# TencentARC/ViT-Lens

Hardware: AMD Instinct MI355X
Metric: modality-pairs/sec (ViT-L, 224^2 patches) (higher is better)
Workload: dtype bf16; 1 GPU; C3: ViT-L Lens(depth)->ViT + image + text tri-modal InfoNCE TRAINING step (fwd+bwd+AdamW), batch 1024/GPU in micro-batches of 256, first 4 blocks + adapter trainable; global_batch=1024, residual_dtype=bf16, accumulate=fp32, parallelism=dp1, gemm_cfg=-1, via=step, text_tower_operands=fp16, layernorm=folded into the GEMMs (frozen blocks), frozen_towers=second HIP stream beside the trainable tower's forward, backward=two halves of the micro-batches on two HIP streams

## Files before the change

include/vitlens_hip.h:

```cpp
#ifndef VITLENS_HIP_H
#define VITLENS_HIP_H

#include <stdint.h>

#ifdef __cplusplus
extern "C" {
#endif

#ifndef __HIP_PLATFORM_AMD__
typedef struct ihipStream_t* hipStream_t;
#endif

#define VL_EPI_BF16 0
#define VL_EPI_F32 1
#define VL_EPI_RES_F32 2
#define VL_EPI_RES_BF16 3
#define VL_EPI_GEGLU 5
#define VL_EPI_DGELU 6
#define VL_EPI_DGEGLU 7
#define VL_ACT_NONE 0
#define VL_ACT_GELU 1
#define VL_ACT_RELU 2
#define VL_ACT_GELU_DSAVE 4
#define VL_ACT_QGELU 5
// ... 100 lines not shown
int vl_transpose_to_bf16(const void* in, int in_dtype, long ldi, int R, int C, void* out, long ldo, hipStream_t stream);
int vl_transpose_colsum_bf16(const void* in, int in_dtype, long ldi, int R, int C, void* out, long ldo,
                             float* colsum_out, float colsum_scale, float* ws, hipStream_t stream);

int vl_split_bf16x3(const float* x, void* out, long rows, int D, int pattern, hipStream_t stream);
int vl_ce_stats(const float* logits, long ld, int R, int C, int label_off, float* row_lse, float* col_lse,
                float* diag, float* col_ws, hipStream_t stream);
int vl_ce_loss_accum(const float* row_lse, const float* col_lse, const float* diag, int R, int C, int label_off,
                     float w_row, float w_col, float* loss_inout, hipStream_t stream);
int vl_ce_grad(const float* logits, long ld, int R, int C, int label_off, const float* row_lse, const float* col_lse,
               float w_row, float w_col, void* G, long ldg, void* GT, long ldgt, float logit_scale,
               float* dscale_inout, float* ws, hipStream_t stream);
long vl_ce_grad_ws_floats(int R, int C, long ldg, long ldgt);
int vl_ce_stats_masked(const float* logits, long ld, int R, int C, int label_off, float* row_lse, float* col_lse,
                       float* diag, float* col_ws, const float* sim, long ld_sim, float thres, hipStream_t stream);
int vl_ce_grad_masked(const float* logits, long ld, int R, int C, int label_off, const float* row_lse, const float* col_lse,
                      float w_row, float w_col, void* G, long ldg, void* GT, long ldgt, float logit_scale,
                      float* dscale_inout, float* ws, const float* sim, long ld_sim, float thres, hipStream_t stream);

int vl_layernorm_bwd(const void* dy, int dy_dtype, long dy_stride, const void* x, int x_dtype, long x_stride,
                     const float* mean, const float* rstd, const float* w, const float* dres, float* dx,
                     void* dx_bf16, long dx_stride, int rows, int D, hipStream_t stream);
int vl_layernorm_bwd_g(const void* dy, int dy_dtype, long dy_stride, const void* x, int x_dtype, long x_stride,
                       const float* mean, const float* rstd, const float* w, const void* dres, void* dx, int g_dtype,
                       void* dx_bf16, long dx_stride, int rows, int D, hipStream_t stream);
int vl_layernorm_bwd_sres(const void* dy, int dy_dtype, long dy_stride, const void* x, int x_dtype, long x_stride,
                          const float* mean, const float* rstd, const float* w, const void* dres, int dres_every,
                          long dres_stride, void* dx, int g_dtype, void* dx_bf16, long dx_stride, int rows, int D,
                          hipStream_t stream);
long vl_colreduce_ws_floats(int rows, int cols, int planes);
int vl_layernorm_bwd_params(const void* dy, int dy_dtype, long dy_stride, const void* x, int x_dtype, long x_stride,
                            const float* mean, const float* rstd, float* dw, float* db, int rows, int D,
                            float* ws, hipStream_t stream);
int vl_colsum(const void* a, int a_dtype, long lda, float* out, int rows, int cols, float scale, float* ws, hipStream_t stream);
int vl_gelu_bf16(const void* u, void* y, long n, hipStream_t stream);
int vl_geglu_bf16(const void* h, void* y, long rows, int n_out, hipStream_t stream);
int vl_attn_bwd_bf16(const void* q, const void* k, const void* v, const void* dO, const void* o, const long* strides,
                     const float* lse, float* delta, void* dq, void* dk, void* dv, long ld_dq, long ld_dkv,
                     int B, int H, int Lq, int Lk, int dh, float qscale, int causal, float scale, hipStream_t stream);
int vl_attn_bwd_fused_supported(int Lq, int Lk, int dh, int causal);
int vl_attn_bwd_fused_bf16(const void* q, const void* k, const void* v, const void* dO, const void* o, const long* strides,
                           const float* lse, void* dq, void* dk, void* dv, long ld_dq, long ld_dkv, int B, int H, int L, int dh,
                           float qscale, float scale, hipStream_t stream);
int vl_attn_fwd_q1(const void* q, const void* k, const void* v, const long* strides, void* out, long ld_out, float* lse,
                   int B, int H, int L, int dh, int qrow, float qscale, hipStream_t stream);
int vl_attn_bwd_q1(const void* q, const void* k, const void* v, const long* strides, const void* dO, long ld_do,
                   const void* o, long ld_o, const float* lse, void* dq, void* dk, void* dv, long ld_dq, long ld_dkv,
                   int B, int H, int L, int dh, int qrow, float qscale, float scale, hipStream_t stream);
int vl_attn_fwd_drop_bf16(const void* q, const void* k, const void* v, const long* strides, void* out, float* lse, int B, int H,
                          int Lq, int Lk, int dh, float qscale, int causal, double p, uint64_t seed, int64_t sample0,
                          int sublayer, hipStream_t stream);
int vl_attn_bwd_drop_bf16(const void* q, const void* k, const void* v, const void* dO, const void* o, const long* strides,
                          const float* lse, float* delta, void* dq, void* dk, void* dv, long ld_dq, long ld_dkv, int B, int H,
                          int Lq, int Lk, int dh, float qscale, int causal, float scale, double p, uint64_t seed,
                          int64_t sample0, int sublayer, hipStream_t stream);
int vl_ff_drop_fwd(const float* y, const float* x0, float* x1, int B, int n, int D, double p, uint64_t seed, int64_t sample0,
                   int sublayer, hipStream_t stream);
int vl_ff_drop_bwd(const float* dx1, void* dy, float* dy_f32, int B, int n, int D, double p, uint64_t seed, int64_t sample0,
                   int sublayer, hipStream_t stream);
int vl_kaldi_fbank(const float* wave, long wave_stride, int batch, long n_samples, const float* window, const float* banks,
                   float* out, int target_len, int win, int shift, int nfft, int nmel, float preemph, float mean, float std,
                   hipStream_t stream);
int vl_resample_sinc(const float* in, long in_stride, int batch, long n_in, const int* offsets, const float* taps, int o, int n,
                     int K, float* out, long out_stride, long out_first, long n_out, hipStream_t stream);
int vl_fbank_augment(const float* in, float* out, int batch, int T, int F, const void* params, float mean, float std,
                     hipStream_t stream);
// ... 112 lines not shown
```

vit-lens_amd/csrc/vl_bwd.hip:

```cpp
#include "vl_common.h"
#include "vitlens_hip.h"

namespace {

__device__ __forceinline__ float ld1(const float* p) { return *p; }
__device__ __forceinline__ float ld1(const bf16_t* p) { return bf2f(*p); }

__device__ __forceinline__ void ld4(const float* p, float (&v)[4]) {
  const f32x4 t = *(const f32x4*)p; v[0] = t[0]; v[1] = t[1]; v[2] = t[2]; v[3] = t[3];
}
__device__ __forceinline__ void ld4(const bf16_t* p, float (&v)[4]) {
  const u32x2 t = *(const u32x2*)p;
  v[0] = bf2f((bf16_t)(t[0] & 0xffff)); v[1] = bf2f((bf16_t)(t[0] >> 16));
  v[2] = bf2f((bf16_t)(t[1] & 0xffff)); v[3] = bf2f((bf16_t)(t[1] >> 16));
}
__device__ __forceinline__ void st4(float* p, const float (&v)[4]) { f32x4 t = {v[0], v[1], v[2], v[3]}; *(f32x4*)p = t; }
__device__ __forceinline__ void st4(bf16_t* p, const float (&v)[4]) {
  u32x2 t; t[0] = pack2bf(v[0], v[1]); t[1] = pack2bf(v[2], v[3]); *(u32x2*)p = t;
}

struct LnBwdP {
  const void* dy; const void* x; const float* mean; const float* rstd; const float* w;
  const void* dres;
  void* dx; bf16_t* dxb;
// ... 41 lines not shown
    }
    s1 = wave_sum(s1) / (float)D; s2 = wave_sum(s2) / (float)D;
#pragma unroll
    for (int c = 0; c < NV; ++c) {
      if (HALF && c == NCH && !tail) break;
      const int e = c * 256 + lane * 4;
      float v[4];
#pragma unroll
      for (int k = 0; k < 4; ++k) v[k] = rs * (g[c][k] - s1 - xh[c][k] * s2);
      if (dres) {
        float r[4]; ld4(dres + e, r);
#pragma unroll
        for (int k = 0; k < 4; ++k) v[k] += r[k];
      }
      if (dx) st4(dx + e, v);
      if (dxb) st4(dxb + e, v);
    }
  } else {
    float s1 = 0.f, s2 = 0.f;
    for (int e = lane; e < D; e += 64) {
      const float g = ld1(dy + e) * p.w[e];
      const float xh = (ld1(x + e) - mu) * rs;
      s1 += g; s2 = fmaf(g, xh, s2);
    }
    s1 = wave_sum(s1) / (float)D; s2 = wave_sum(s2) / (float)D;
    for (int e = lane; e < D; e += 64) {
      const float g = ld1(dy + e) * p.w[e];
      const float xh = (ld1(x + e) - mu) * rs;
      float v = rs * (g - s1 - xh * s2);
      if (dres) v += ld1(dres + e);
      if (dx) { if constexpr (sizeof(TG) == 4) dx[e] = v; else dx[e] = f2bf(v); }
      if (dxb) dxb[e] = f2bf(v);
    }
  }
}

__global__ void __launch_bounds__(256) gelu_kernel(const bf16_t* u, bf16_t* y, long n) {
  for (long i = ((long)blockIdx.x * 256 + threadIdx.x) * 8; i < n; i += (long)gridDim.x * 256 * 8) {
    const u32x4 v = *(const u32x4*)(u + i);
    u32x4 o;
#pragma unroll
    for (int e = 0; e < 4; ++e)
      o[e] = pack2bf(gelu_erf(bf2f((bf16_t)(v[e] & 0xffff))), gelu_erf(bf2f((bf16_t)(v[e] >> 16))));
    *(u32x4*)(y + i) = o;
  }
}

__global__ void __launch_bounds__(256) geglu_kernel(const bf16_t* h, bf16_t* y, long n) {
  for (long i = ((long)blockIdx.x * 256 + threadIdx.x) * 4; i < n; i += (long)gridDim.x * 256 * 4) {
    const u32x4 v = *(const u32x4*)(h + 2 * i);
    u32x2 o;
    o[0] = pack2bf(bf2f((bf16_t)(v[0] & 0xffff)) * gelu_erf(bf2f((bf16_t)(v[0] >> 16))),
                   bf2f((bf16_t)(v[1] & 0xffff)) * gelu_erf(bf2f((bf16_t)(v[1] >> 16))));
    o[1] = pack2bf(bf2f((bf16_t)(v[2] & 0xffff)) * gelu_erf(bf2f((bf16_t)(v[2] >> 16))),
                   bf2f((bf16_t)(v[3] & 0xffff)) * gelu_erf(bf2f((bf16_t)(v[3] >> 16))));
    *(u32x2*)(y + i) = o;
  }
}

struct AdamwC { float lr, b1, b2, eps, bc1, bc2_sqrt; };
__device__ __forceinline__ void adamw_update(float& pi, const float gi, float& mi, float& vi, const AdamwC c, const float wd) {
#pragma clang fp contract(off)
  const float decay = fmaf(-c.lr, wd, 1.0f);
  mi = fmaf(1.0f - c.b1, gi, c.b1 * mi);
  vi = c.b2 * vi + ((1.0f - c.b2) * gi) * gi;
  pi = pi * decay - ((c.lr / c.bc1) * mi) / (sqrtf(vi) / c.bc2_sqrt + c.eps);
// ... 177 lines not shown
  else if (vec && p.D == 256) hipLaunchKernelGGL((ln_bwd_kernel<1, TDY, TX, TG>), g, b, 0, stream, p);
  else hipLaunchKernelGGL((ln_bwd_kernel<0, TDY, TX, TG>), g, b, 0, stream, p);
}

static int ln_bwd_run(const void* dy, int dy_dtype, long dy_stride, const void* x, int x_dtype, long x_stride,
                      const float* mean, const float* rstd, const float* w, const void* dres, int dres_every, long dres_stride,
                      void* dx, int g_dtype, void* dx_bf16, long dx_stride, int rows, int D, hipStream_t stream) {
  if (rows <= 0 || D <= 0) return vl_set_error("vl_layernorm_bwd: empty problem");
  for (const int dt : {dy_dtype, x_dtype, g_dtype})
    if (dt != VL_F32 && dt != VL_BF16) return vl_set_error("vl_layernorm_bwd: dy_dtype, x_dtype and g_dtype must be VL_F32 or VL_BF16");
  LnBwdP p{dy, x, mean, rstd, w, dres, dx, (bf16_t*)dx_bf16, dy_stride, x_stride, dx_stride, rows, D, dres_every, dres_stride};
  const int key = (dy_dtype == VL_BF16 ? 4 : 0) | (x_dtype == VL_BF16 ? 2 : 0) | (g_dtype == VL_BF16 ? 1 : 0);
  switch (key) {
    case 0: ln_bwd_launch<float, float, float>(p, stream); break;
    case 1: ln_bwd_launch<float, float, bf16_t>(p, stream); break;
    case 2: ln_bwd_launch<float, bf16_t, float>(p, stream); break;
    case 3: ln_bwd_launch<float, bf16_t, bf16_t>(p, stream); break;
    case 4: ln_bwd_launch<bf16_t, float, float>(p, stream); break;
    case 5: ln_bwd_launch<bf16_t, float, bf16_t>(p, stream); break;
    case 6: ln_bwd_launch<bf16_t, bf16_t, float>(p, stream); break;
    default: ln_bwd_launch<bf16_t, bf16_t, bf16_t>(p, stream); break;
  }
  VL_HIP_OK(hipGetLastError());
  return 0;
}

extern "C" int vl_layernorm_bwd_g(const void* dy, int dy_dtype, long dy_stride, const void* x, int x_dtype, long x_stride,
                                  const float* mean, const float* rstd, const float* w, const void* dres, void* dx, int g_dtype,
                                  void* dx_bf16, long dx_stride, int rows, int D, hipStream_t stream) {
  return ln_bwd_run(dy, dy_dtype, dy_stride, x, x_dtype, x_stride, mean, rstd, w, dres, 1, dx_stride, dx, g_dtype, dx_bf16, dx_stride,
                    rows, D, stream);
}

extern "C" int vl_layernorm_bwd_sres(const void* dy, int dy_dtype, long dy_stride, const void* x, int x_dtype, long x_stride,
                                     const float* mean, const float* rstd, const float* w, const void* dres, int dres_every,
                                     long dres_stride, void* dx, int g_dtype, void* dx_bf16, long dx_stride, int rows, int D,
                                     hipStream_t stream) {
  if (!dres || !dx || dres_every < 1) return vl_set_error("vl_layernorm_bwd_sres: dres, dx and dres_every >= 1 are required");
  if (dres == dx) return vl_set_error("vl_layernorm_bwd_sres: dres must not alias dx");
  return ln_bwd_run(dy, dy_dtype, dy_stride, x, x_dtype, x_stride, mean, rstd, w, dres, dres_every, dres_stride, dx, g_dtype, dx_bf16,
                    dx_stride, rows, D, stream);
}

extern "C" int vl_layernorm_bwd(const void* dy, int dy_dtype, long dy_stride, const void* x, int x_dtype, long x_stride,
                                const float* mean, const float* rstd, const float* w, const float* dres, float* dx,
                                void* dx_bf16, long dx_stride, int rows, int D, hipStream_t stream) {
  return vl_layernorm_bwd_g(dy, dy_dtype, dy_stride, x, x_dtype, x_stride, mean, rstd, w, dres, dx, VL_F32, dx_bf16, dx_stride, rows, D, stream);
}

extern "C" int vl_gelu_bf16(const void* u, void* y, long n, hipStream_t stream) {
  if (n <= 0) return 0;
  if (n & 7) return vl_set_error("vl_gelu_bf16: n must be a multiple of 8");
  hipLaunchKernelGGL(gelu_kernel, dim3(grid_for(n / 8)), dim3(256), 0, stream, (const bf16_t*)u, (bf16_t*)y, n);
  VL_HIP_OK(hipGetLastError());
  return 0;
}

extern "C" int vl_geglu_bf16(const void* h, void* y, long rows, int n_out, hipStream_t stream) {
  const long n = rows * n_out;
  if (n <= 0) return 0;
  if (n_out & 3) return vl_set_error("vl_geglu_bf16: n_out must be a multiple of 4");
  hipLaunchKernelGGL(geglu_kernel, dim3(grid_for(n / 4)), dim3(256), 0, stream, (const bf16_t*)h, (bf16_t*)y, n);
  VL_HIP_OK(hipGetLastError());
  return 0;
}

// ... 69 lines not shown
```

vit-lens_amd/csrc/vl_colreduce.hip:

```cpp
#include "vl_common.h"
#include "vitlens_hip.h"

namespace {

template <int V, typename T>
__device__ __forceinline__ void ldv(const T* p, float (&f)[V]) {
  constexpr bool kF32 = sizeof(T) == 4;
  static_assert(V == 1 || (kF32 ? V == 4 : V == 4 || V == 8), "no load of this width");
  if constexpr (V == 1) {
    if constexpr (kF32) f[0] = *p; else f[0] = bf2f(*p);
  } else if constexpr (kF32) {
    const f32x4 v = *(const f32x4*)p;
#pragma unroll
    for (int e = 0; e < 4; ++e) f[e] = v[e];
  } else {
    typedef __attribute__((ext_vector_type(V / 2))) unsigned int words_t;
    const words_t v = *(const words_t*)p;
#pragma unroll
    for (int e = 0; e < V / 2; ++e) { f[2 * e] = bf2f((bf16_t)(v[e] & 0xffff)); f[2 * e + 1] = bf2f((bf16_t)(v[e] >> 16)); }
  }
}

template <int V, int NR, int U, bool LN, typename TA, typename TX>
__global__ void __launch_bounds__(256) colreduce_kernel(const TA* a, long lda, const TX* x, long xs, const float* mean,
// ... 71 lines not shown
  if (j < D) {
    for (int r = r0 + ry; r < r1; r += 8) {
      const bool two = r + 4 < r1;
      const int r2 = two ? r + 4 : r;
      const u32x2 g0 = *(const u32x2*)(dy + (long)r * dys + j), g1 = *(const u32x2*)(dy + (long)r2 * dys + j);
      const f32x4 x0 = *(const f32x4*)(x + (long)r * xs + j), x1 = *(const f32x4*)(x + (long)r2 * xs + j);
      const float m0 = mean[r], s0 = rstd[r], m1 = mean[r2], s1 = two ? rstd[r2] : 0.f;
      const float k1 = two ? 1.f : 0.f;
#pragma unroll
      for (int e = 0; e < 4; ++e) {
        const float gl = bf2f((bf16_t)((e & 1) ? (g0[e >> 1] >> 16) : (g0[e >> 1] & 0xffff)));
        const float hl = bf2f((bf16_t)((e & 1) ? (g1[e >> 1] >> 16) : (g1[e >> 1] & 0xffff)));
        a[e] = fmaf(gl, (x0[e] - m0) * s0, a[e]);
        b[e] += gl;
        a[e] = fmaf(hl, (x1[e] - m1) * s1, a[e]);
        b[e] = fmaf(hl, k1, b[e]);
      }
    }
  }
  if (ry) {
#pragma unroll
    for (int e = 0; e < 4; ++e) { sh[ry - 1][cx][e] = a[e]; sh[ry - 1][cx][4 + e] = b[e]; }
  }
  __syncthreads();
  if (ry == 0 && j < D) {
#pragma unroll
    for (int e = 0; e < 4; ++e) {
      ws[((long)blockIdx.y * 2) * D + j + e] = (a[e] + sh[0][cx][e]) + (sh[1][cx][e] + sh[2][cx][e]);
      ws[((long)blockIdx.y * 2 + 1) * D + j + e] = (b[e] + sh[0][cx][4 + e]) + (sh[1][cx][4 + e] + sh[2][cx][4 + e]);
    }
  }
}

__global__ void __launch_bounds__(1024) slab_finalize_kernel(const float* ws, int nslab, int K, int D, float scale, float* out0, float* out1) {
  __shared__ float sh[16][64];
  const int jl = threadIdx.x & 63, g = threadIdx.x >> 6;
  const int j = blockIdx.x * 64 + jl, k = blockIdx.y;
  float s = 0.f;
  if (j < D)
    for (int t = g; t < nslab; t += 16) s += ws[((long)t * K + k) * D + j];
  sh[g][jl] = s;
  __syncthreads();
  if (g == 0 && j < D) {
    float a[16];
#pragma unroll
    for (int i = 0; i < 16; ++i) a[i] = sh[i][jl];
#pragma unroll
    for (int w = 8; w > 0; w >>= 1)
#pragma unroll
      for (int i = 0; i < w; ++i) a[i] += a[i + w];
    float* o = k == 0 ? out0 : out1;
    o[j] += a[0] * scale;
  }
}

}

extern "C" int vl_set_error(const char* msg);
#define VL_HIP_OK(e) do { hipError_t _e = (e); if (_e != hipSuccess) return vl_set_error(hipGetErrorString(_e)); } while (0)

static const int kSlabRows = 256;
extern "C" long vl_colreduce_ws_floats(int rows, int cols, int planes) {
  return (long)((rows + kSlabRows - 1) / kSlabRows) * planes * cols;
}

template <typename T>
static bool vec_ok(int V, const void* p, long stride, int cols) {
  return cols % V == 0 && stride % V == 0 && (uintptr_t)p % (V * sizeof(T)) == 0;
}

template <int V, int NR, int U, bool LN, typename TA, typename TX>
static void stage1_launch(const void* a, long lda, const void* x, long xs, const float* mean, const float* rstd, float* ws,
                          int rows, int cols, int nslab, hipStream_t stream) {
  constexpr int per_block = 256 / NR * V;
  hipLaunchKernelGGL((colreduce_kernel<V, NR, U, LN, TA, TX>), dim3((cols + per_block - 1) / per_block, nslab), dim3(256), 0, stream,
                     (const TA*)a, lda, (const TX*)x, xs, mean, rstd, ws, rows, cols, kSlabRows);
}

template <int V, bool LN, typename TA, typename TX>
static void colreduce_launch(const void* a, long lda, const void* x, long xs, const float* mean, const float* rstd, float* ws,
                             int rows, int cols, float scale, float* out0, float* out1, hipStream_t stream) {
  const int nslab = (rows + kSlabRows - 1) / kSlabRows;
  bool vec = false;
  if constexpr (V > 1) {
    vec = vec_ok<TA>(V, a, lda, cols) && (!LN || vec_ok<TX>(V, x, xs, cols));
    if constexpr (LN && V == 4) {
      if (vec)
        hipLaunchKernelGGL(ln_bwd_params4_bf16_f32_kernel, dim3((cols + 255) / 256, nslab), dim3(256), 0, stream, (const bf16_t*)a, lda,
                           (const float*)x, xs, mean, rstd, ws, rows, cols, kSlabRows);
    } else if (vec) {
      stage1_launch<V, 4, LN ? 2 : 4, LN, TA, TX>(a, lda, x, xs, mean, rstd, ws, rows, cols, nslab, stream);
    }
  }
  if (!vec) stage1_launch<1, 1, 1, LN, TA, TX>(a, lda, x, xs, mean, rstd, ws, rows, cols, nslab, stream);
  hipLaunchKernelGGL(slab_finalize_kernel, dim3((cols + 63) / 64, LN ? 2 : 1), dim3(1024), 0, stream, ws, nslab, LN ? 2 : 1, cols,
                     scale, out0, out1);
}

extern "C" int vl_layernorm_bwd_params(const void* dy, int dy_dtype, long dy_stride, const void* x, int x_dtype, long x_stride,
                                       const float* mean, const float* rstd, float* dw, float* db, int rows, int D,
                                       float* ws, hipStream_t stream) {
  if (rows <= 0 || D <= 0) return vl_set_error("vl_layernorm_bwd_params: empty problem");
  if (!ws) return vl_set_error("vl_layernorm_bwd_params: workspace of vl_colreduce_ws_floats(rows, D, 2) floats required");
#define VL_LN_PARAMS(V, TA, TX) colreduce_launch<V, true, TA, TX>(dy, dy_stride, x, x_stride, mean, rstd, ws, rows, D, 1.0f, dw, db, stream)
  if (dy_dtype == VL_BF16 && x_dtype == VL_F32) VL_LN_PARAMS(4, bf16_t, float);
  else if (dy_dtype == VL_BF16) VL_LN_PARAMS(8, bf16_t, bf16_t);
  else if (x_dtype == VL_F32) VL_LN_PARAMS(1, float, float);
  else VL_LN_PARAMS(1, float, bf16_t);
#undef VL_LN_PARAMS
  VL_HIP_OK(hipGetLastError());
  return 0;
}

extern "C" int vl_colsum(const void* a, int a_dtype, long lda, float* out, int rows, int cols, float scale, float* ws, hipStream_t stream) {
  if (rows <= 0 || cols <= 0) return vl_set_error("vl_colsum: empty problem");
  if (!ws) return vl_set_error("vl_colsum: workspace of vl_colreduce_ws_floats(rows, cols, 1) floats required");
  if (a_dtype == VL_BF16) colreduce_launch<8, false, bf16_t, bf16_t>(a, lda, nullptr, 0, nullptr, nullptr, ws, rows, cols, scale, out, out, stream);
  else colreduce_launch<4, false, float, float>(a, lda, nullptr, 0, nullptr, nullptr, ws, rows, cols, scale, out, out, stream);
  VL_HIP_OK(hipGetLastError());
  return 0;
}
```

vit-lens_amd/vitlens_hip/_lib.py:

```python
import ctypes as C
import os

_HERE = os.path.dirname(os.path.abspath(__file__))
_LIB = None


class LibraryNotBuilt(ImportError):
    pass


def lib_path() -> str:
    return os.path.join(_HERE, "libvitlens_hip.so")


P, I, L, F = C.c_void_p, C.c_int, C.c_long, C.c_float

ABI_VERSION = 610

SIGNATURES = {
    "vl_version": [],
    "vl_device_info": [I, C.c_char_p, I, C.POINTER(I), C.POINTER(I), C.POINTER(L)],
    "vl_gemm_bf16": [P, P, P, P, P, I, I, I, I, I, I, F, I, I, I, P],
    "vl_gemm_splitk_accum_f32": [P, P, P, I, I, I, I, I, L, F, I, P, P],
    "vl_gemm_tn_splitk_accum_f32": [P, P, P, I, I, I, I, I, L, F, I, P, P],
# ... 42 lines not shown
    "vl_fbank_augment": [P, P, I, I, I, P, F, F, P],
    "vl_wave_clip_mix": [P, L, P, P, P, I, L, P],
    "vl_mix_rows": [P, P, P, P, P, I, L, P],
    "vl_fps": [P, P, P, P, I, I, I, P],
    "vl_pc_gather_normalize": [P, P, P, I, I, I, I, P],
    "vl_pc_augment": [P, P, P, I, I, I, I, P, F, P],
    "vl_rgbd_augment": [P, I, I, I, P, P, P, P, F, F, F, P, P, P],
    "vl_image_crop_resize_u8": [P, I, I, I, P, P, P, P],
    "vl_image_augment": [P, I, I, I, I, P, P, P, P, P, P, P, P],
    "vl_tactile_augment": [P, I, I, I, P, P, P, P, P, P],
    "vl_resample_h_u8": [P, L, I, I, I, I, P, P, I, I, I, P, P],
    "vl_resample_v_u8_norm": [P, I, I, I, I, P, P, I, I, I, P, P, P, P, P],
    "vl_resample_batch_u8_norm": [P, I, I, I, I, I, P, P, P, P, P, P],
    "vl_resample_h_f32": [P, L, I, I, I, P, P, I, I, I, I, F, F, F, P, P],
    "vl_resample_v_f32_norm": [P, I, I, I, P, P, I, I, I, F, F, P, P],
    "vl_knn_group": [P, P, P, P, I, I, I, I, I, P],
    "vl_ball_group": [P, P, P, P, P, I, I, I, I, F, I, I, P],
    "vl_group_max": [P, L, P, I, L, L, I, I, P],
    "vl_pad3_bf16": [P, P, L, I, P],
    "vl_bn_stats": [P, L, I, I, P, I, P, P, P, P, F, P],
    "vl_bn_stats_local": [P, L, I, I, P, I, P, P],
    "vl_bn_stats_merge": [P, I, I, P, P, P, P, F, P, P],
    "vl_bn_bwd_reduce": [P, L, P, L, P, P, P, P, F, I, P, I, P, P, P, I, I, P],
    "vl_bn_bwd_apply": [P, L, P, L, P, P, P, P, F, I, P, P, P, L, I, I, P],
    "vl_bn_apply": [P, L, P, P, P, P, F, I, P, L, L, I, P],
    "vl_bn_bwd": [P, L, P, L, P, P, P, P, F, I, I, P, I, P, P, P, L, I, I, P],
    "vl_group_max_bwd": [P, L, P, L, P, L, P, L, L, I, I, P],
    "vl_group_sum": [P, L, P, L, L, I, I, P],
    "vl_layernorm_bwd": [P, I, L, P, I, L, P, P, P, P, P, P, L, I, I, P],
    "vl_layernorm_bwd_g": [P, I, L, P, I, L, P, P, P, P, P, I, P, L, I, I, P],
    "vl_layernorm_bwd_sres": [P, I, L, P, I, L, P, P, P, P, I, L, P, I, P, L, I, I, P],
    "vl_colreduce_ws_floats": [I, I, I],
    "vl_layernorm_bwd_params": [P, I, L, P, I, L, P, P, P, P, I, I, P, P],
    "vl_colsum": [P, I, L, P, I, I, F, P, P],
    "vl_gelu_bf16": [P, P, L, P],
    "vl_geglu_bf16": [P, P, L, I, P],
    "vl_attn_bwd_bf16": [P, P, P, P, P, P, P, P, P, P, P, L, L, I, I, I, I, I, F, I, F, P],
    "vl_attn_bwd_fused_supported": [I, I, I, I],
    "vl_attn_bwd_fused_bf16": [P, P, P, P, P, P, P, P, P, P, L, L, I, I, I, I, F, F, P],
    "vl_attn_fwd_q1": [P, P, P, P, P, L, P, I, I, I, I, I, F, P],
    "vl_attn_bwd_q1": [P, P, P, P, P, L, P, L, P, P, P, P, L, L, I, I, I, I, I, F, F, P],
    "vl_adamw_step": [P, P, P, P, L, F, F, F, F, F, I, F, P],
    "vl_sumsq_ws_floats": [],
    "vl_sumsq_f32": [P, L, P, P, P],
    "vl_adamw_multi_step": [P, I, F, F, F, F, I, F, F, P, P, P],
    "vl_clamp_scalar": [P, F, F, P],
    "vl_axpy_f32": [P, P, F, L, P],
    "vl_scale_exp_f32": [P, P, L, P, F, P],
    "vl_batch_rowsum": [P, P, I, I, I, L, L, P],
    "vl_attn_fwd_drop_bf16": [P, P, P, P, P, P, I, I, I, I, I, F, I, C.c_double, C.c_uint64, C.c_int64, I, P],
    "vl_attn_bwd_drop_bf16": [P, P, P, P, P, P, P, P, P, P, P, L, L, I, I, I, I, I, F, I, F, C.c_double, C.c_uint64, C.c_int64, I, P],
    "vl_ff_drop_fwd": [P, P, P, I, I, I, C.c_double, C.c_uint64, C.c_int64, I, P],
    "vl_ff_drop_bwd": [P, P, P, I, I, I, C.c_double, C.c_uint64, C.c_int64, I, P],
    "vl_lp_bn_fwd": [P, L, P, F, C.c_uint64, C.c_int64, I, P, P, F, F, P, L, P, L, P, P, I, I, P],
    "vl_ce_label_ws_floats": [I, I],
    "vl_ce_label": [P, L, P, I, I, F, P, P, L, P, L, P, P, P],
    "vl_lars_ws_floats": [L, I],
    "vl_lars_multi_step": [P, I, F, F, F, F, F, P, P, L, P],
    "vl_topk_hits": [P, L, P, I, I, I, I, P, P, P],
    "vl_eval_hits": [P, L, P, P, I, I, I, I, P, P, P, P, P, P],
    "vl_average_precision_ws_bytes": [I, I],
    "vl_average_precision": [P, L, P, L, I, I, P, P, P],
    "vl_clip_mean_normalize": [P, L, I, I, I, F, P, P],
    "vl_comm_unique_id": [P],
    "vl_comm_create": [C.POINTER(P), P, I, I],
    "vl_comm_destroy": [P],
# ... 44 lines not shown
```

vit-lens_amd/vitlens_hip/ops.py:

```python
import ctypes as C
import threading

import numpy as np
import torch

from ._lib import load_library, check

F32, BF16, F16 = 0, 1, 2
EPI_BF16, EPI_F32, EPI_RES_F32, EPI_RES_BF16, EPI_GEGLU, EPI_DGELU, EPI_DGEGLU = 0, 1, 2, 3, 5, 6, 7
ACT_NONE, ACT_GELU, ACT_RELU = 0, 1, 2
ACT_GELU_DSAVE = 4
ACT_QGELU = 5
ACT_QGELU_DSAVE = 6


def mlp_act(quick_gelu: bool, dsave: bool = False) -> int:
    if quick_gelu:
        return ACT_QGELU_DSAVE if dsave else ACT_QGELU
    return ACT_GELU_DSAVE if dsave else ACT_GELU
LOG2E = 1.4426950408889634

_lib = load_library()


# ... 629 lines not shown
                                     sim.stride(0), float(thres), _stream()))
    return G, GT


def device_info(device=0):
    arch = C.create_string_buffer(64)
    cus, clk, mem = C.c_int(), C.c_int(), C.c_long()
    check(_lib.vl_device_info(device, arch, 64, C.byref(cus), C.byref(clk), C.byref(mem)))
    return {"arch": arch.value.decode(), "cus": cus.value, "clock_khz": clk.value, "hbm_bytes": mem.value}


def layernorm_bwd(dy, x, mean, rstd, w, rows, D, dres=None, dx=None, dx_bf16=None, x_row_stride=None,
                  dy_row_stride=None, dx_row_stride=None):
    g = dx if dx is not None else dres
    gdt = F32 if g is None else _dt(g)
    if dres is not None and dx is not None and dres.dtype != dx.dtype:
        raise TypeError("layernorm_bwd: dres and dx must share a dtype")
    check(_lib.vl_layernorm_bwd_g(_p(dy), _dt(dy), D if dy_row_stride is None else dy_row_stride, _p(x), _dt(x),
                                  D if x_row_stride is None else x_row_stride, _p(mean), _p(rstd), _p(w), _p(dres),
                                  _p(dx), gdt, _p(dx_bf16), D if dx_row_stride is None else dx_row_stride, rows, D, _stream()))


def layernorm_bwd_sparse_res(dy, x, mean, rstd, w, rows, D, dres, dres_every, dx):
    if dres.dtype != dx.dtype or dres.dim() != 2 or dres.stride(1) != 1 or dres.shape[0] * dres_every < rows - dres_every + 1:
        raise ValueError("layernorm_bwd_sparse_res: dres must be a row-major matrix of dx's dtype with one row per dres_every rows")
    check(_lib.vl_layernorm_bwd_sres(_p(dy), _dt(dy), D, _p(x), _dt(x), D, _p(mean), _p(rstd), _p(w), _p(dres), int(dres_every),
                                     dres.stride(0), _p(dx), _dt(dx), None, D, rows, D, _stream()))


_colreduce_ws = {}


def _ws_for(device, rows, cols, planes):
    need = int(_lib.vl_colreduce_ws_floats(rows, cols, planes))
    key = (device, torch.cuda.current_stream(device).cuda_stream, threading.get_ident())
    t = _colreduce_ws.get(key)
    if t is None or t.numel() < need:
        t = torch.empty(need, device=device, dtype=torch.float32)
        _colreduce_ws[key] = t
    return t


def layernorm_bwd_params(dy, x, mean, rstd, dw, db, rows, D, x_row_stride=None, dy_row_stride=None):
    ws = _ws_for(dy.device, rows, D, 2)
    check(_lib.vl_layernorm_bwd_params(_p(dy), _dt(dy), D if dy_row_stride is None else dy_row_stride, _p(x), _dt(x),
                                       D if x_row_stride is None else x_row_stride, _p(mean), _p(rstd), _p(dw), _p(db),
                                       rows, D, _p(ws), _stream()))


def colsum(a, out, scale=1.0):
    _chk2d(a, "a")
    ws = _ws_for(a.device, a.shape[0], a.shape[1], 1)
    check(_lib.vl_colsum(_p(a), _dt(a), a.stride(0), _p(out), a.shape[0], a.shape[1], float(scale), _p(ws), _stream()))


def geglu_bf16(h, out):
    check(_lib.vl_geglu_bf16(_p(h), _p(out), h.shape[0], h.shape[1] // 2, _stream()))
    return out


def gelu_bf16(u, out):
    check(_lib.vl_gelu_bf16(_p(u), _p(out), u.numel(), _stream()))
    return out


def attn_bwd(q, k, v, dO, o, lse, delta, dq, dk, dv, ld_dq, ld_dkv, causal=False, softmax_scale=None, qscale=None, fused=None):
    B, H, Lq, dh = q.shape
    Lk = k.shape[2]
    scale = dh ** -0.5 if softmax_scale is None else softmax_scale
    qs = scale * LOG2E if qscale is None else qscale
    st = _bhld_strides(q, k, v, dO, o)
    if fused is None:
        fused = bool(_lib.vl_attn_bwd_fused_supported(Lq, Lk, dh, 1 if causal else 0))
    if fused:
        if Lq != Lk or causal:
            raise ValueError("attn_bwd(fused=True): self-attention without a causal mask only")
        check(_lib.vl_attn_bwd_fused_bf16(_p(q), _p(k), _p(v), _p(dO), _p(o), st, _p(lse), _p(dq), _p(dk), _p(dv),
                                          ld_dq, ld_dkv, B, H, Lq, dh, float(qs), float(scale), _stream()))
        return
    check(_lib.vl_attn_bwd_bf16(_p(q), _p(k), _p(v), _p(dO), _p(o), st, _p(lse), _p(delta), _p(dq), _p(dk), _p(dv),
# ... 756 lines not shown
```

vit-lens_amd/vitlens_hip/train.py:

```python
from typing import Dict, Iterable, Optional

import torch

from . import ops
from . import engine as _engine
from .engine import VitEngine, deinterleave_geglu

BF = torch.bfloat16


class _Saved:

    def __init__(self, B, L, D, H, hidden, layers, device, res_dtype=torch.float32, keep_blocks=(), checkpoint=False):
        dh = D // H
        T = B * L
        Lp = (L + 7) // 8 * 8
        f32 = lambda *s: torch.empty(*s, device=device, dtype=torch.float32)
        bf = lambda *s: torch.empty(*s, device=device, dtype=BF)
        self.Lp = Lp
        xres = f32 if res_dtype == torch.float32 else bf

        def per_layer(make):
            if not checkpoint:
                return [make() for _ in range(layers)]
            one = make()
            return [one] * layers
        mids = per_layer(lambda: xres(T, D))
        self.X = [None] * (2 * layers + 1)
        for l in range(layers):
            self.X[2 * l] = xres(T, D); self.X[2 * l + 1] = mids[l]
        self.X[2 * layers] = xres(T, D)
        ident = lambda: [torch.zeros(T, device=device), torch.ones(T, device=device), torch.zeros(T, device=device),
                         torch.ones(T, device=device)]
        self.stats = per_layer(ident)
        self.qkv = per_layer(lambda: bf(T, 3 * D))
        hv = lambda m, i=0: ops.heads_view(m, B, L, H, dh, i * D)
        self.q = [hv(m, 0) for m in self.qkv]; self.k = [hv(m, 1) for m in self.qkv]; self.v = [hv(m, 2) for m in self.qkv]
        self.a = per_layer(lambda: bf(T, D))
        self.av = [hv(m) for m in self.a]
        self.lse = per_layer(lambda: f32(B, H, L))
        self.u = per_layer(lambda: bf(T, hidden))
# ... 163 lines not shown
        if self._drop is not None:
            dtok = ops.scatter_rows_keep(dxpre, self._drop[1], L - 1)
            if self.train_pos:
                gpos = self.grad_buffer(P + "positional_embedding", e.pos)
                ops.batch_rowsum(dxpre, gpos[:1], B, 1, D, L, 0)
                ops.batch_rowsum(dtok, gpos[1:], B, T, D, T, 0)
            return dtok
        if self.train_pos:
            ops.batch_rowsum(dxpre, self.grad_buffer(P + "positional_embedding", e.pos), B, L, D, L, 0)
        return dxpre.view(B, L, D)[:, 1:, :].reshape(B * T, D)

    def _cls_block_backward(self, S, l, B, L):
        e, D = self.eng, self.D
        w, wT, cfg = e.blocks[l], self.wT[l], e.gemm_cfg
        m1, r1 = S.stats[l][0], S.stats[l][1]
        x1c = _engine.cls_rows(S.X[2 * l + 1], B, L)
        ops.gemm(S.dxc, wT["proj_w"], None, out=S.du1, res=S.u1, epi=ops.EPI_DGELU, act=self.act_dsave, cfg=cfg)
        ops.gemm(S.du1, wT["fc_w"], None, out=S.dhc, epi=ops.EPI_BF16, cfg=cfg)
        ops.layernorm_bwd(S.dhc, x1c, S.stats2c[0], S.stats2c[1], w["ln2_w"], B, D, dres=S.dxc, dx=S.dxc, x_row_stride=L * D)
        ops.gemm(S.dxc, wT["out_w"], None, out=S.dO1, epi=ops.EPI_BF16, cfg=cfg)
        ops.attn_bwd_q1(S.q[l], S.k[l], S.v[l], S.dO1, S.a1, S.lse1, S.dqkv, S.dqkv[:, D:], S.dqkv[:, 2 * D:], 3 * D, 3 * D, qrow=0)
        ops.gemm(S.dqkv, wT["in_w"], None, out=S.dh, epi=ops.EPI_BF16, cfg=cfg)
        ops.layernorm_bwd_sparse_res(S.dh, S.X[2 * l], m1, r1, w["ln1_w"], B * L, D, dres=S.dxc, dres_every=L, dx=S.dx)

    def _blocks_backward(self, S, B, L, on_block_done=None, cls_only=False):
        e, D, H = self.eng, self.D, self.H
        rows = B * L
        cfg = e.gemm_cfg
        P = self.prefix
        f32_stream = S.dx.dtype == torch.float32
        dxb_out = S.dxb if f32_stream else None
        if f32_stream:
            ops.cast_bf16(S.dx, out=S.dxb)
        for l in reversed(range(self.layers)):
            if cls_only and l == self.layers - 1:
                self._cls_block_backward(S, l, B, L)
                continue
            if self.checkpoint:
                self._block_forward(S, l, B, L, write_out=False)
            w, wT = e.blocks[l], self.wT[l]
            m1, r1, m2, r2 = S.stats[l]
            trainable = l in self.train_blocks
            bp = f"{P}transformer.resblocks.{l}."
            ops.gemm(S.dxb, wT["proj_w"], None, out=S.du, res=S.u[l], epi=ops.EPI_DGELU, act=self.act_dsave, cfg=cfg)
            if trainable:
                self._dw(bp + "mlp.c_proj.weight", S.dx, S.hidk[l], bp + "mlp.c_proj.bias")
                self._dw(bp + "mlp.c_fc.weight", S.du, S.h2[l], bp + "mlp.c_fc.bias")
            ops.gemm(S.du, wT["fc_w"], None, out=S.dh, epi=ops.EPI_BF16, cfg=cfg)
            if trainable:
                ops.layernorm_bwd_params(S.dh, S.X[2 * l + 1], m2, r2, self.grad_buffer(bp + "ln_2.weight", w["ln2_w"]),
                                         self.grad_buffer(bp + "ln_2.bias", w["ln2_b"]), rows, D)
            ops.layernorm_bwd(S.dh, S.X[2 * l + 1], m2, r2, w["ln2_w"], rows, D, dres=S.dx, dx=S.dx, dx_bf16=dxb_out)
            if trainable:
                self._dw(bp + "attn.out_proj.weight", S.dx, S.a[l], bp + "attn.out_proj.bias")
            ops.gemm(S.dxb, wT["out_w"], None, out=S.dOm, epi=ops.EPI_BF16, cfg=cfg)
            ops.attn_bwd(S.q[l], S.k[l], S.v[l], S.dO, S.av[l], S.lse[l], S.delta,
                         S.dqkv, S.dqkv[:, D:], S.dqkv[:, 2 * D:], 3 * D, 3 * D, causal=self.causal)
            if trainable:
                self._dw(bp + "attn.in_proj_weight", S.dqkv, S.h1[l], bp + "attn.in_proj_bias")
            ops.gemm(S.dqkv, wT["in_w"], None, out=S.dh, epi=ops.EPI_BF16, cfg=cfg)
            if trainable:
                ops.layernorm_bwd_params(S.dh, S.X[2 * l], m1, r1, self.grad_buffer(bp + "ln_1.weight", w["ln1_w"]),
                                         self.grad_buffer(bp + "ln_1.bias", w["ln1_b"]), rows, D)
            ops.layernorm_bwd(S.dh, S.X[2 * l], m1, r1, w["ln1_w"], rows, D, dres=S.dx, dx=S.dx, dx_bf16=dxb_out)
            if trainable and on_block_done is not None:
                on_block_done(l)


def conv_weight_grad(dtok: torch.Tensor, cols: torch.Tensor, g: torch.Tensor, gemm_cfg: int = -1):
    ops.weight_grad(ops.cast_bf16(dtok.contiguous()), cols, g, cfg=gemm_cfg)


class DepthLensTrainer:

    def __init__(self, lens_engine, unlock_first_n: int = 4, tower_kw=None):
        self.le = lens_engine
        kw = dict(train_blocks=range(unlock_first_n)) if tower_kw is None else dict(tower_kw)
        self.tower = TowerTrainer(lens_engine.vit, param_prefix="visual.", **kw)
        self.ctx = None

    @property
    def grads(self):
        return self.tower.grads

    def forward(self, x: torch.Tensor, keep=None, inv=None) -> torch.Tensor:
        le = self.le
        cols = le.cols(x)
        tok = ops.gemm(cols, le.conv_w, None, epi=ops.EPI_BF16, cfg=le.gemm_cfg)
        self.ctx = (cols, x.shape[0])
        return self.tower.forward(tok, x.shape[0], pos2=le.adapter_pos, keep=keep, inv=inv)

    def backward(self, dfeat: torch.Tensor, on_block_done=None):
        cols, B = self.ctx
        dtok = self.tower.backward(dfeat, on_block_done)
        T, D = dtok.shape[0] // B, dtok.shape[1]
        t = self.tower
        g = t.grad_buffer("visual.visual_adapter.conv1.weight_gemm", torch.empty(D, cols.shape[1]))
# ... 451 lines not shown
```

Baseline: 1884 modality-pairs/sec.

## Fuse LayerNorm backward with its param-grad and next bias column sums

Adds a single LayerNorm-backward kernel that writes dx and, in the same pass, accumulates per-column partial sums for ln weight/bias grads and the column sum of the resulting dx. That dx column sum is the bias grad of the preceding linear layer (out_proj or the block below's c_proj). The trainer uses it for trainable blocks, so the separate layernorm_bwd_params pass and the bias column reductions inside _dw are skipped. This cuts extra reads of dy, x and dx over all rows. In exchange it adds a partial-sum workspace, a finalize launch, and bookkeeping across blocks for which c_proj bias was already produced.

```diff
diff --git a/include/vitlens_hip.h b/include/vitlens_hip.h
--- a/include/vitlens_hip.h
+++ b/include/vitlens_hip.h
@@ -156,6 +156,10 @@
 int vl_layernorm_bwd_params(const void* dy, int dy_dtype, long dy_stride, const void* x, int x_dtype, long x_stride,
                             const float* mean, const float* rstd, float* dw, float* db, int rows, int D,
                             float* ws, hipStream_t stream);
+int vl_layernorm_bwd_sums_parts(int rows, int D);
+int vl_layernorm_bwd_sums(const void* dy, long dy_stride, const void* x, int x_dtype, long x_stride, const float* mean,
+                          const float* rstd, const float* w, const void* dres, void* dx, int g_dtype, void* dx_bf16,
+                          long dx_stride, float* dw, float* db, float* dcol, int rows, int D, float* ws, hipStream_t stream);
 int vl_colsum(const void* a, int a_dtype, long lda, float* out, int rows, int cols, float scale, float* ws, hipStream_t stream);
 int vl_gelu_bf16(const void* u, void* y, long n, hipStream_t stream);
 int vl_geglu_bf16(const void* h, void* y, long rows, int n_out, hipStream_t stream);
diff --git a/vit-lens_amd/csrc/vl_bwd.hip b/vit-lens_amd/csrc/vl_bwd.hip
--- a/vit-lens_amd/csrc/vl_bwd.hip
+++ b/vit-lens_amd/csrc/vl_bwd.hip
@@ -97,6 +97,97 @@
       if (dx) { if constexpr (sizeof(TG) == 4) dx[e] = v; else dx[e] = f2bf(v); }
       if (dxb) dxb[e] = f2bf(v);
     }
+  }
+}
+
+constexpr int kLnSumsWaves = 4;
+template <typename T> struct Raw4 { typedef f32x4 type; };
+template <> struct Raw4<bf16_t> { typedef u32x2 type; };
+template <int NCH, typename TX, typename TG>
+__global__ void __launch_bounds__(kLnSumsWaves * 64) __attribute__((amdgpu_waves_per_eu(3))) ln_bwd_sums_kernel(const LnBwdP p, float* ws, const int want) {
+#pragma clang fp contract(off)
+  __shared__ float sh[kLnSumsWaves - 1][NCH * 256];
+  const int lane = threadIdx.x & 63, wv = threadIdx.x >> 6;
+  const long gw = (long)blockIdx.x * kLnSumsWaves + wv, nw = (long)gridDim.x * kLnSumsWaves;
+  const int r0 = (int)(gw * p.rows / nw), r1 = (int)((gw + 1) * p.rows / nw);
+  const int D = p.D;
+  const bool round_dx = sizeof(TG) == 2 || !p.dx;
+  float acc[3][NCH][4];
+#pragma unroll
+  for (int a = 0; a < 3; ++a)
+#pragma unroll
+    for (int c = 0; c < NCH; ++c)
+#pragma unroll
+      for (int k = 0; k < 4; ++k) acc[a][c][k] = 0.f;
+  for (int row = r0; row < r1; ++row) {
+    const bf16_t* dy = (const bf16_t*)p.dy + (long)row * p.dys;
+    const TX* x = (const TX*)p.x + (long)row * p.xs;
+    const TG* dres = p.dres ? (const TG*)p.dres + (long)row * p.dxs : nullptr;
+    TG* dx = p.dx ? (TG*)p.dx + (long)row * p.dxs : nullptr;
+    bf16_t* dxb = p.dxb ? p.dxb + (long)row * p.dxs : nullptr;
+    const float mu = p.mean[row], rs = p.rstd[row];
+    float g[NCH][4], xh[NCH][4], d0[4], w0[4];
+    float s1 = 0.f, s2 = 0.f;
+    typename Raw4<TG>::type rr[NCH];
+    if (dres) {
+#pragma unroll
+      for (int c = 0; c < NCH; ++c) rr[c] = *(const typename Raw4<TG>::type*)(dres + c * 256 + lane * 4);
+    }
+#pragma unroll
+    for (int c = 0; c < NCH; ++c) {
+      const int e = c * 256 + lane * 4;
+      float d[4], ww[4];
+      ld4(dy + e, d); ld4(x + e, xh[c]); ld4(p.w + e, ww);
+#pragma unroll
+      for (int k = 0; k < 4; ++k) {
+        g[c][k] = d[k] * ww[k]; xh[c][k] = (xh[c][k] - mu) * rs;
+        s1 += g[c][k]; s2 = fmaf(g[c][k], xh[c][k], s2);
+        acc[0][c][k] = fmaf(d[k], xh[c][k], acc[0][c][k]); acc[1][c][k] += d[k];
+        if (c == 0) { d0[k] = d[k]; w0[k] = ww[k]; }
+      }
+    }
+    s1 = wave_sum(s1) / (float)D; s2 = wave_sum(s2) / (float)D;
+#pragma unroll
+    for (int c = 0; c < NCH; ++c) {
+      const int e = c * 256 + lane * 4;
+      float v[4];
+#pragma unroll
+      for (int k = 0; k < 4; ++k) v[k] = rs * fmaf(-s2, xh[c][k], c == 0 ? fmaf(d0[k], w0[k], -s1) : g[c][k] - s1);
+      if (dres) {
+        float r[4]; ld4((const TG*)&rr[c], r);
+#pragma unroll
+        for (int k = 0; k < 4; ++k) v[k] += r[k];
+      }
+      if (dx) st4(dx + e, v);
+      if (dxb) st4(dxb + e, v);
+#pragma unroll
+      for (int k = 0; k < 4; ++k) acc[2][c][k] += round_dx ? bf2f(f2bf(v[k])) : v[k];
+    }
+  }
+  int slot = 0;
+#pragma unroll
+  for (int a = 0; a < 3; ++a) {
+    if (!(want >> a & 1)) continue;
+    if (wv > 0) {
+#pragma unroll
+      for (int c = 0; c < NCH; ++c) st4(&sh[wv - 1][c * 256 + lane * 4], acc[a][c]);
+    }
+    __syncthreads();
+    if (wv == 0) {
+      float* out = ws + ((long)blockIdx.x * __popc(want) + slot) * D;
+#pragma unroll
+      for (int c = 0; c < NCH; ++c) {
+        float s[4] = {acc[a][c][0], acc[a][c][1], acc[a][c][2], acc[a][c][3]};
+        for (int w = 0; w < kLnSumsWaves - 1; ++w) {
+          float t[4]; ld4(&sh[w][c * 256 + lane * 4], t);
+#pragma unroll
+          for (int k = 0; k < 4; ++k) s[k] += t[k];
+        }
+        st4(out + c * 256 + lane * 4, s);
+      }
+    }
+    __syncthreads();
+    ++slot;
   }
 }
 
@@ -340,6 +431,56 @@
                     rows, D, stream);
 }
 
+void vl_colreduce_finalize(const float* ws, int nparts, int planes, int cols, float* out0, float* out1, float* out2, hipStream_t stream);
+
+extern "C" int vl_layernorm_bwd_sums_parts(int rows, int D) {
+  if (rows <= 0 || D <= 0 || D % 256 != 0 || D > 1024) return 0;
+  const int n = (rows + kLnSumsWaves - 1) / kLnSumsWaves;
+  return n > 768 ? 768 : n;
+}
+
+template <typename TX, typename TG>
+static void ln_bwd_sums_launch(const LnBwdP& p, float* ws, int want, int nparts, hipStream_t stream) {
+  const dim3 g(nparts), b(kLnSumsWaves * 64);
+  switch (p.D / 256) {
+    case 1: hipLaunchKernelGGL((ln_bwd_sums_kernel<1, TX, TG>), g, b, 0, stream, p, ws, want); break;
+    case 2: hipLaunchKernelGGL((ln_bwd_sums_kernel<2, TX, TG>), g, b, 0, stream, p, ws, want); break;
+    case 3: hipLaunchKernelGGL((ln_bwd_sums_kernel<3, TX, TG>), g, b, 0, stream, p, ws, want); break;
+    default: hipLaunchKernelGGL((ln_bwd_sums_kernel<4, TX, TG>), g, b, 0, stream, p, ws, want); break;
+  }
+}
+
+extern "C" int vl_layernorm_bwd_sums(const void* dy, long dy_stride, const void* x, int x_dtype, long x_stride, const float* mean,
+                                     const float* rstd, const float* w, const void* dres, void* dx, int g_dtype, void* dx_bf16,
+                                     long dx_stride, float* dw, float* db, float* dcol, int rows, int D, float* ws,
+                                     hipStream_t stream) {
+  const int nparts = vl_layernorm_bwd_sums_parts(rows, D);
+  if (nparts == 0) return vl_set_error("vl_layernorm_bwd_sums: D must be 256, 512, 768 or 1024 and rows > 0 (vl_layernorm_bwd_sums_parts)");
+  for (const int dt : {x_dtype, g_dtype})
+    if (dt != VL_F32 && dt != VL_BF16) return vl_set_error("vl_layernorm_bwd_sums: x_dtype and g_dtype must be VL_F32 or VL_BF16");
+  const int want = (dw ? 1 : 0) | (db ? 2 : 0) | (dcol ? 4 : 0);
+  if (!want) return vl_set_error("vl_layernorm_bwd_sums: none of dw, db, dcol is given (vl_layernorm_bwd_g is the plain form)");
+  if (!ws) return vl_set_error("vl_layernorm_bwd_sums: workspace of vl_layernorm_bwd_sums_parts(rows, D) * 3 * D floats required");
+  if (!dx && !dx_bf16) return vl_set_error("vl_layernorm_bwd_sums: dx or dx_bf16 is required");
+  const size_t eg = g_dtype == VL_BF16 ? 2 : 4;
+  auto al4 = [](const void* q, size_t elem) { return (uintptr_t)q % (4 * elem) == 0; };
+  if (dy_stride % 4 || x_stride % 4 || dx_stride % 4 || !al4(dy, 2) || !al4(x, x_dtype == VL_BF16 ? 2 : 4) || !al4(w, 4) ||
+      !al4(dres, eg) || !al4(dx, eg) || !al4(dx_bf16, 2) || !al4(ws, 4))
+    return vl_set_error("vl_layernorm_bwd_sums: every row stride and base address must be a multiple of 4 elements");
+  LnBwdP p{dy, x, mean, rstd, w, dres, dx, (bf16_t*)dx_bf16, dy_stride, x_stride, dx_stride, rows, D, 1, dx_stride};
+  switch ((x_dtype == VL_BF16 ? 2 : 0) | (g_dtype == VL_BF16 ? 1 : 0)) {
+    case 0: ln_bwd_sums_launch<float, float>(p, ws, want, nparts, stream); break;
+    case 1: ln_bwd_sums_launch<float, bf16_t>(p, ws, want, nparts, stream); break;
+    case 2: ln_bwd_sums_launch<bf16_t, float>(p, ws, want, nparts, stream); break;
+    default: ln_bwd_sums_launch<bf16_t, bf16_t>(p, ws, want, nparts, stream); break;
+  }
+  float* outs[3]; int n = 0;
+  for (float* o : {dw, db, dcol}) if (o) outs[n++] = o;
+  vl_colreduce_finalize(ws, nparts, n, D, outs[0], n > 1 ? outs[1] : nullptr, n > 2 ? outs[2] : nullptr, stream);
+  VL_HIP_OK(hipGetLastError());
+  return 0;
+}
+
 extern "C" int vl_layernorm_bwd_sres(const void* dy, int dy_dtype, long dy_stride, const void* x, int x_dtype, long x_stride,
                                      const float* mean, const float* rstd, const float* w, const void* dres, int dres_every,
                                      long dres_stride, void* dx, int g_dtype, void* dx_bf16, long dx_stride, int rows, int D,
diff --git a/vit-lens_amd/csrc/vl_colreduce.hip b/vit-lens_amd/csrc/vl_colreduce.hip
--- a/vit-lens_amd/csrc/vl_colreduce.hip
+++ b/vit-lens_amd/csrc/vl_colreduce.hip
@@ -127,7 +127,8 @@
   }
 }
 
-__global__ void __launch_bounds__(1024) slab_finalize_kernel(const float* ws, int nslab, int K, int D, float scale, float* out0, float* out1) {
+__global__ void __launch_bounds__(1024) slab_finalize_kernel(const float* ws, int nslab, int K, int D, float scale, float* out0, float* out1,
+                                                             float* out2) {
   __shared__ float sh[16][64];
   const int jl = threadIdx.x & 63, g = threadIdx.x >> 6;
   const int j = blockIdx.x * 64 + jl, k = blockIdx.y;
@@ -144,7 +145,7 @@
     for (int w = 8; w > 0; w >>= 1)
 #pragma unroll
       for (int i = 0; i < w; ++i) a[i] += a[i + w];
-    float* o = k == 0 ? out0 : out1;
+    float* o = k == 0 ? out0 : k == 1 ? out1 : out2;
     o[j] += a[0] * scale;
   }
 }
@@ -189,7 +190,12 @@
   }
   if (!vec) stage1_launch<1, 1, 1, LN, TA, TX>(a, lda, x, xs, mean, rstd, ws, rows, cols, nslab, stream);
   hipLaunchKernelGGL(slab_finalize_kernel, dim3((cols + 63) / 64, LN ? 2 : 1), dim3(1024), 0, stream, ws, nslab, LN ? 2 : 1, cols,
-                     scale, out0, out1);
+                     scale, out0, out1, nullptr);
+}
+
+void vl_colreduce_finalize(const float* ws, int nparts, int planes, int cols, float* out0, float* out1, float* out2, hipStream_t stream) {
+  hipLaunchKernelGGL(slab_finalize_kernel, dim3((cols + 63) / 64, planes), dim3(1024), 0, stream, ws, nparts, planes, cols, 1.0f, out0,
+                     out1, out2);
 }
 
 extern "C" int vl_layernorm_bwd_params(const void* dy, int dy_dtype, long dy_stride, const void* x, int x_dtype, long x_stride,
diff --git a/vit-lens_amd/vitlens_hip/_lib.py b/vit-lens_amd/vitlens_hip/_lib.py
--- a/vit-lens_amd/vitlens_hip/_lib.py
+++ b/vit-lens_amd/vitlens_hip/_lib.py
@@ -98,6 +98,8 @@
     "vl_layernorm_bwd_sres": [P, I, L, P, I, L, P, P, P, P, I, L, P, I, P, L, I, I, P],
     "vl_colreduce_ws_floats": [I, I, I],
     "vl_layernorm_bwd_params": [P, I, L, P, I, L, P, P, P, P, I, I, P, P],
+    "vl_layernorm_bwd_sums_parts": [I, I],
+    "vl_layernorm_bwd_sums": [P, L, P, I, L, P, P, P, P, P, I, P, L, P, P, P, I, I, P, P],
     "vl_colsum": [P, I, L, P, I, I, F, P, P],
     "vl_gelu_bf16": [P, P, L, P],
     "vl_geglu_bf16": [P, P, L, I, P],
diff --git a/vit-lens_amd/vitlens_hip/ops.py b/vit-lens_amd/vitlens_hip/ops.py
--- a/vit-lens_amd/vitlens_hip/ops.py
+++ b/vit-lens_amd/vitlens_hip/ops.py
@@ -685,7 +685,10 @@
 
 
 def _ws_for(device, rows, cols, planes):
-    need = int(_lib.vl_colreduce_ws_floats(rows, cols, planes))
+    return _ws_floats(device, int(_lib.vl_colreduce_ws_floats(rows, cols, planes)))
+
+
+def _ws_floats(device, need):
     key = (device, torch.cuda.current_stream(device).cuda_stream, threading.get_ident())
     t = _colreduce_ws.get(key)
     if t is None or t.numel() < need:
@@ -699,6 +702,25 @@
     check(_lib.vl_layernorm_bwd_params(_p(dy), _dt(dy), D if dy_row_stride is None else dy_row_stride, _p(x), _dt(x),
                                        D if x_row_stride is None else x_row_stride, _p(mean), _p(rstd), _p(dw), _p(db),
                                        rows, D, _p(ws), _stream()))
+
+
+def layernorm_bwd_sums_ok(D):
+    return int(_lib.vl_layernorm_bwd_sums_parts(1, int(D))) > 0
+
+
+def layernorm_bwd_sums(dy, x, mean, rstd, w, rows, D, dres=None, dx=None, dx_bf16=None, dw=None, db=None, dcol=None):
+    g = dx if dx is not None else dres
+    gdt = F32 if g is None else _dt(g)
+    if dres is not None and dx is not None and dres.dtype != dx.dtype:
+        raise TypeError("layernorm_bwd_sums: dres and dx must share a dtype")
+    for name, t in (("dw", dw), ("db", db), ("dcol", dcol)):
+        if t is not None and (t.dtype != torch.float32 or t.numel() != D or not t.is_contiguous()):
+            raise ValueError(f"layernorm_bwd_sums: {name} must be a contiguous f32 tensor of {D} elements")
+    ws = _ws_floats(dy.device, int(_lib.vl_layernorm_bwd_sums_parts(rows, D)) * 3 * D)
+    if dy.dtype != torch.bfloat16:
+        raise TypeError("layernorm_bwd_sums: dy must be bf16 (layernorm_bwd + layernorm_bwd_params + colsum take an fp32 dy)")
+    check(_lib.vl_layernorm_bwd_sums(_p(dy), dy.stride(0), _p(x), _dt(x), x.stride(0), _p(mean), _p(rstd), _p(w),
+                                     _p(dres), _p(dx), gdt, _p(dx_bf16), D, _p(dw), _p(db), _p(dcol), rows, D, _p(ws), _stream()))
 
 
 def colsum(a, out, scale=1.0):
diff --git a/vit-lens_amd/vitlens_hip/train.py b/vit-lens_amd/vitlens_hip/train.py
--- a/vit-lens_amd/vitlens_hip/train.py
+++ b/vit-lens_amd/vitlens_hip/train.py
@@ -7,6 +7,8 @@
 from .engine import VitEngine, deinterleave_geglu
 
 BF = torch.bfloat16
+
+FUSE_PARAM_SUMS = True
 
 
 class _Saved:
@@ -236,9 +238,12 @@
         dxb_out = S.dxb if f32_stream else None
         if f32_stream:
             ops.cast_bf16(S.dx, out=S.dxb)
+        fuse = bool(FUSE_PARAM_SUMS and self.train_blocks and ops.layernorm_bwd_sums_ok(D))
+        cproj_bias_done = False
         for l in reversed(range(self.layers)):
             if cls_only and l == self.layers - 1:
                 self._cls_block_backward(S, l, B, L)
+                cproj_bias_done = False
                 continue
             if self.checkpoint:
                 self._block_forward(S, l, B, L, write_out=False)
@@ -248,25 +253,39 @@
             bp = f"{P}transformer.resblocks.{l}."
             ops.gemm(S.dxb, wT["proj_w"], None, out=S.du, res=S.u[l], epi=ops.EPI_DGELU, act=self.act_dsave, cfg=cfg)
             if trainable:
-                self._dw(bp + "mlp.c_proj.weight", S.dx, S.hidk[l], bp + "mlp.c_proj.bias")
+                self._dw(bp + "mlp.c_proj.weight", S.dx, S.hidk[l], None if cproj_bias_done else bp + "mlp.c_proj.bias")
                 self._dw(bp + "mlp.c_fc.weight", S.du, S.h2[l], bp + "mlp.c_fc.bias")
             ops.gemm(S.du, wT["fc_w"], None, out=S.dh, epi=ops.EPI_BF16, cfg=cfg)
+            if trainable and fuse:
+                ops.layernorm_bwd_sums(S.dh, S.X[2 * l + 1], m2, r2, w["ln2_w"], rows, D, dres=S.dx, dx=S.dx, dx_bf16=dxb_out,
+                                       dw=self.grad_buffer(bp + "ln_2.weight", w["ln2_w"]),
+                                       db=self.grad_buffer(bp + "ln_2.bias", w["ln2_b"]),
+                                       dcol=self.grad_buffer(bp + "attn.out_proj.bias", w["ln2_b"]))
+            else:
+                if trainable:
+                    ops.layernorm_bwd_params(S.dh, S.X[2 * l + 1], m2, r2, self.grad_buffer(bp + "ln_2.weight", w["ln2_w"]),
+                                             self.grad_buffer(bp + "ln_2.bias", w["ln2_b"]), rows, D)
+                ops.layernorm_bwd(S.dh, S.X[2 * l + 1], m2, r2, w["ln2_w"], rows, D, dres=S.dx, dx=S.dx, dx_bf16=dxb_out)
             if trainable:
-                ops.layernorm_bwd_params(S.dh, S.X[2 * l + 1], m2, r2, self.grad_buffer(bp + "ln_2.weight", w["ln2_w"]),
-                                         self.grad_buffer(bp + "ln_2.bias", w["ln2_b"]), rows, D)
-            ops.layernorm_bwd(S.dh, S.X[2 * l + 1], m2, r2, w["ln2_w"], rows, D, dres=S.dx, dx=S.dx, dx_bf16=dxb_out)
-            if trainable:
-                self._dw(bp + "attn.out_proj.weight", S.dx, S.a[l], bp + "attn.out_proj.bias")
+                self._dw(bp + "attn.out_proj.weight", S.dx, S.a[l], None if fuse else bp + "attn.out_proj.bias")
             ops.gemm(S.dxb, wT["out_w"], None, out=S.dOm, epi=ops.EPI_BF16, cfg=cfg)
             ops.attn_bwd(S.q[l], S.k[l], S.v[l], S.dO, S.av[l], S.lse[l], S.delta,
                          S.dqkv, S.dqkv[:, D:], S.dqkv[:, 2 * D:], 3 * D, 3 * D, causal=self.causal)
             if trainable:
                 self._dw(bp + "attn.in_proj_weight", S.dqkv, S.h1[l], bp + "attn.in_proj_bias")
             ops.gemm(S.dqkv, wT["in_w"], None, out=S.dh, epi=ops.EPI_BF16, cfg=cfg)
-            if trainable:
-                ops.layernorm_bwd_params(S.dh, S.X[2 * l], m1, r1, self.grad_buffer(bp + "ln_1.weight", w["ln1_w"]),
-                                         self.grad_buffer(bp + "ln_1.bias", w["ln1_b"]), rows, D)
-            ops.layernorm_bwd(S.dh, S.X[2 * l], m1, r1, w["ln1_w"], rows, D, dres=S.dx, dx=S.dx, dx_bf16=dxb_out)
+            cproj_bias_done = fuse and (l - 1) in self.train_blocks
+            if fuse and (trainable or cproj_bias_done):
+                below = f"{P}transformer.resblocks.{l - 1}.mlp.c_proj.bias"
+                ops.layernorm_bwd_sums(S.dh, S.X[2 * l], m1, r1, w["ln1_w"], rows, D, dres=S.dx, dx=S.dx, dx_bf16=dxb_out,
+                                       dw=self.grad_buffer(bp + "ln_1.weight", w["ln1_w"]) if trainable else None,
+                                       db=self.grad_buffer(bp + "ln_1.bias", w["ln1_b"]) if trainable else None,
+                                       dcol=self.grad_buffer(below, w["ln1_b"]) if cproj_bias_done else None)
+            else:
+                if trainable:
+                    ops.layernorm_bwd_params(S.dh, S.X[2 * l], m1, r1, self.grad_buffer(bp + "ln_1.weight", w["ln1_w"]),
+                                             self.grad_buffer(bp + "ln_1.bias", w["ln1_b"]), rows, D)
+                ops.layernorm_bwd(S.dh, S.X[2 * l], m1, r1, w["ln1_w"], rows, D, dres=S.dx, dx=S.dx, dx_bf16=dxb_out)
             if trainable and on_block_done is not None:
                 on_block_done(l)
 
```

Measured after the change: 1888 modality-pairs/sec (median of 2 runs). Within noise of the previous version (+0.2%).
